# Lynx-MR/orbslam3lib

Measured on AMD Instinct MI355X. Metric: Mfeatures/s extract + Mmatches/s BFMatch, 640x480 stereo 8-level pyr, 1/2/4/8 GPU, higher is better.
Workload: dtype u8; 1 GPU; C2 640x480 stereo, 8 levels x1.2, 2000 feat/frame, FAST 20/7, + per-pair 2000x2000 Hamming kNN2 (left->right, all rows); parallelism=frames sharded across 1 GPU(s), replicas

## Files before the change

### orbslam3lib_amd/csrc/orb_kernels.hip

```cpp
#include <hip/hip_runtime.h>
#include <stdint.h>

#include <algorithm>
#include <atomic>

#include "orb_kernels.h"
#include "orb_math.h"
#include "orb_fast_cell.h"
#include "orb_octree.h"
#include "orb_pattern_data.h"
#include "orb_policy.h"

namespace orbgpu {

static_assert(sizeof(BatchArgs) <= 4096, "kernel argument block too large");

struct PatternTable {
    int8_t v[1024];
};
constexpr int hexval(char c) { return c <= '9' ? c - '0' : c - 'a' + 10; }
constexpr PatternTable make_pattern() {
    PatternTable t{};
    const char* h = ORBGPU_PATTERN_HEX;
    for (int i = 0; i < 1024; ++i) t.v[i] = (int8_t)(hexval(h[2 * i]) * 16 + hexval(h[2 * i + 1]));
// ... 923 lines not shown
        bool bad = false;
#pragma unroll
        for (int k = 0; k < kMaxLevels; ++k)
            if (k < a.nlevels) {
                if (k < l) out_row0 += a.lvlcnt[img * kMaxLevels + k];
                total += a.lvlcnt[img * kMaxLevels + k];
                bad |= a.status[img * kMaxLevels + k] != 0;
            }
        out_ok = !bad && total <= a.out_cap;
        if (bx == 0 && threadIdx.x == 0) {
            a.out_n[img] = bad ? -5 : total > a.out_cap ? -2 : total;
            a.out_mono[img] = out_ok ? total : 0;
        }
    }
    KP28* const out_kp = reinterpret_cast<KP28*>(a.out_kps) + (long long)img * a.out_cap + out_row0;
    uint8_t* const out_d = a.out_desc + ((long long)img * a.out_cap + out_row0) * 32;
    __shared__ __attribute__((aligned(16))) uint4 s_rng[17][17];
    __shared__ __attribute__((aligned(16))) uint4 s_pat[kOdPairs][kOdLanes];
    static_assert(kOdPairs * kOdLanes == 256 && 17 * 17 <= 2 * 256, "table copy: one / two entries per thread");
    const uint4* rng_src = reinterpret_cast<const uint4*>(c_od_tab.rng);
    const uint4 rng0 = rng_src[threadIdx.x];
    const uint4 pat0 = reinterpret_cast<const uint4*>(c_od_tab.pat)[threadIdx.x];
    if (threadIdx.x < 17 * 17 - 256) (&s_rng[0][0])[threadIdx.x + 256] = rng_src[threadIdx.x + 256];
    (&s_rng[0][0])[threadIdx.x] = rng0;
    (&s_pat[0][0])[threadIdx.x] = pat0;
    __syncthreads();
    int mv[3], mlo[3], mhi[3], mofs[3], mp16[3];
#pragma unroll
    for (int it = 0; it < 3; ++it) {
        const int i = sub + 32 * it, r = i / 3, part = i - 3 * r;
        mv[it] = r - 15;
        const int d = r < 31 ? c_umax[mv[it] < 0 ? -mv[it] : mv[it]] : -1;
        mlo[it] = 15 - d - 16 * part;
        mhi[it] = 16 + d - 16 * part;
        mofs[it] = (r < 31 ? mv[it] : 15) * G.pitch + 16 * part;
        mp16[it] = 16 * part;
    }
    const __amdgpu_buffer_rsrc_t lrs =
        __builtin_amdgcn_make_buffer_rsrc((void*)lvl, (short)0, (int)min((long long)G.pitch * G.h, 0x7fffffffLL), 0x00020000);
    uint8_t* pt = patch[grp];
    const int wave_first = (bx - G.od_first) * kOdKpBlock + (threadIdx.x >> 6) * 2;
    auto key_at = [&](int kb) {
        const int kp = kb + (grp & 1);
        return kp < count ? a.lvlkey[kbase + kp] : a.lvlkey[kbase + kb];
    };
    uint32_t key_next = wave_first < count ? key_at(wave_first) : 0u;
    for (int kb = wave_first; kb < count; kb += stride_k) {
        const int kp = kb + (grp & 1);
        const bool valid = kp < count;
        const uint32_t key = key_next;
        if (kb + stride_k < count) key_next = key_at(kb + stride_k);
        const int x = key_x(key) + kMinBorder, y = key_y(key) + kMinBorder;
        const int al = (x - 15) & 15;
        const int wofs = y * G.pitch + (x - 15 - al);
        uint4 mc[3];
#pragma unroll
        for (int it = 0; it < 3; ++it) {
            if (raw_dw) {
                const auto q = __builtin_amdgcn_raw_buffer_load_b128(lrs, wofs + mofs[it], 0, 0);
                mc[it] = make_uint4(q[0], q[1], q[2], q[3]);
            } else {
                const uint8_t* q = lvl + wofs + mofs[it];
                uint32_t d4[4];
#pragma unroll
                for (int k = 0; k < 4; ++k)
                    d4[k] = (uint32_t)q[4 * k] | ((uint32_t)q[4 * k + 1] << 8) | ((uint32_t)q[4 * k + 2] << 16) |
                            ((uint32_t)q[4 * k + 3] << 24);
                mc[it] = make_uint4(d4[0], d4[1], d4[2], d4[3]);
            }
        }
        const int xb = (x - kOdPatchR) & ~3;
        const int pofs = (y - kOdPatchR) * G.bpitch + xb;
        uint4 pv[kOdPatchIt];
#pragma unroll
        for (int it = 0; it < kOdPatchIt; ++it) {
            const int c = sub + it * kOdLanes;
            const int r = c / 3, part = c - 3 * r;
            if (c < kOdPatchChunks) {
                const auto q = __builtin_amdgcn_raw_buffer_load_b128(brs, pofs + r * G.bpitch + 16 * part, 0, 0);
                pv[it] = make_uint4(q[0], q[1], q[2], q[3]);
            }
        }
        int s_all = 0, c_all = 0, m01p = 0;
#pragma unroll
        for (int it = 0; it < 3; ++it) {
            const int m = min(max(mlo[it] + al, 0), 16), n = min(max(mhi[it] + al, 0), 16);
            const uint4 mk = s_rng[m][n];
            const uint32_t p0 = mc[it].x & mk.x, p1 = mc[it].y & mk.y, p2 = mc[it].z & mk.z, p3 = mc[it].w & mk.w;
            uint32_t sc = __builtin_amdgcn_udot4(p0, 0x01010101u, 0u, false);
            sc = __builtin_amdgcn_udot4(p1, 0x01010101u, sc, false);
            sc = __builtin_amdgcn_udot4(p2, 0x01010101u, sc, false);
            sc = __builtin_amdgcn_udot4(p3, 0x01010101u, sc, false);
            uint32_t cc = __builtin_amdgcn_udot4(p0, 0x03020100u, 0u, false);
            cc = __builtin_amdgcn_udot4(p1, 0x07060504u, cc, false);
            cc = __builtin_amdgcn_udot4(p2, 0x0B0A0908u, cc, false);
            cc = __builtin_amdgcn_udot4(p3, 0x0F0E0D0Cu, cc, false);
            s_all += (int)sc;
            c_all += (int)cc + mp16[it] * (int)sc;
            m01p += mv[it] * (int)sc;
        }
        const int m10 = od_sum(c_all - (15 + al) * s_all), m01 = od_sum(m01p);
        const float angle = fast_atan2_deg((float)m01, (float)m10);
        const float factorPI = (float)(3.14159265358979323846 / 180.0);
        float sn, ca;
        libm_sincosf(angle * factorPI, &sn, &ca);
#pragma unroll
        for (int it = 0; it < kOdPatchIt; ++it) {
            const int c = sub + it * kOdLanes;
            const int r = c / 3, part = c - 3 * r;
            if (c < kOdPatchChunks) *reinterpret_cast<uint4*>(pt + r * kOdPatchPitch + 16 * part) = pv[it];
        }
        __builtin_amdgcn_fence(__ATOMIC_RELEASE, "wavefront");
        __builtin_amdgcn_wave_barrier();
        __builtin_amdgcn_fence(__ATOMIC_ACQUIRE, "wavefront");
        const int pc = kOdPatchR * kOdPatchPitch + (x - xb);
        const float magic = 12582912.0f;
        const uint32_t kofs = (uint32_t)pc - 0x4B400000u - 0x400000u * (uint32_t)kOdPatchPitch;
        const f32x2 snv = {sn, sn}, cav = {ca, ca}, mg = {magic, magic};
        typedef const __attribute__((address_space(3))) uint8_t lds_u8;
        const uint32_t kpb = kofs + (uint32_t)(uintptr_t)(lds_u8*)pt;
        uint32_t bits = 0;
#pragma unroll
        for (int b = kOdPairs - 1; b >= 0; --b) {
            uint4 pw = s_pat[b][sub];
            asm volatile("" : "+v"(pw.x), "+v"(pw.y), "+v"(pw.z), "+v"(pw.w));
            const f32x2 X = {__uint_as_float(pw.x), __uint_as_float(pw.y)};
            const f32x2 Y = {__uint_as_float(pw.z), __uint_as_float(pw.w)};
            const f32x2 R = (X * snv + Y * cav) + mg;
            const f32x2 C = (X * cav - Y * snv) + mg;
            uint32_t m0 = __umul24(__float_as_uint(R.x), (uint32_t)kOdPatchPitch) + __float_as_uint(C.x);
            uint32_t m1 = __umul24(__float_as_uint(R.y), (uint32_t)kOdPatchPitch) + __float_as_uint(C.y);
            asm volatile("" : "+v"(m0), "+v"(m1));
            const uint32_t p0 = *(lds_u8*)(uintptr_t)(m0 + kpb), p1 = *(lds_u8*)(uintptr_t)(m1 + kpb);
            bits = __builtin_amdgcn_bitop3_b32(bits, (p0 - p1) >> (31 - b), 1u << b, 0xf8);
        }
        if (valid && !out_ok) {
            if (sub == 0) a.lvlangle[kbase + kp] = angle;
            a.lvldesc[(kbase + kp) * 32 + sub] = (uint8_t)bits;
        }
        if (valid) {
            if (out_ok) {
                out_d[kp * 32 + sub] = (uint8_t)bits;
                if (sub < 7) {
                    float px = (float)(x), py = (float)(y);
                    if (l != 0) {
                        px = px * G.scale;
                        py = py * G.scale;
                    }
                    const uint32_t w7[7] = {__float_as_uint(px), __float_as_uint(py), __float_as_uint((float)G.patch),
                                            __float_as_uint(angle), __float_as_uint((float)key_resp(key)),
                                            (uint32_t)l, 0xFFFFFFFFu};
                    uint32_t v = w7[0];
#pragma unroll
                    for (int k = 1; k < 7; ++k) v = sub == k ? w7[k] : v;
                    reinterpret_cast<uint32_t*>(out_kp + kp)[sub] = v;
                }
            }
        }
    }
}


constexpr int kFinU = 2;
#ifndef FIN_WIDE_MAX
#define FIN_WIDE_MAX 8
#endif
constexpr int kFinWideMaxImages = FIN_WIDE_MAX;

template <int kFinThreads>
__global__ __launch_bounds__(kFinThreads) void k_finalize(BatchArgs a) {
    __shared__ int4 s_lv[kMaxLevels];
    __shared__ int s_wave[2][kFinThreads / 64];
    const int img = a.img0 + blockIdx.x;
    const int tid = threadIdx.x, lane = tid & 63, w = tid >> 6;
    const int L = a.nlevels;
    int off[kMaxLevels];
    int total = 0;
    bool bad = false;
#pragma unroll
    for (int l = 0; l < kMaxLevels; ++l) {
        off[l] = total;
        if (l < L) {
            total += a.lvlcnt[img * kMaxLevels + l];
            bad |= a.status[img * kMaxLevels + l] != 0;
        }
    }
    if (bad || total > a.out_cap) {
        if (tid == 0) {
            a.out_n[img] = bad ? -5 : -2;
            a.out_mono[img] = 0;
        }
        return;
    }
    if (tid == 0) {
#pragma unroll
        for (int l = 0; l < kMaxLevels; ++l)
            if (l < L) s_lv[l] = make_int4(a.lv[l].kp_off, off[l], __float_as_int(l == 0 ? 1.f : a.lv[l].scale), a.lv[l].patch);
    }
    __syncthreads();
    const float lap0 = (float)a.laps[2 * img], lap1 = (float)a.laps[2 * img + 1];
    KP28* out = reinterpret_cast<KP28*>(a.out_kps) + (long long)img * a.out_cap;
    uint8_t* od = a.out_desc + (long long)img * a.out_cap * 32;
    const long long ibase = (long long)img * a.lvlkp_img_stride;
    const uint64_t lt = (1ull << lane) - 1ull;
    int mono = 0, stereo = 0, chunk_no = 0;
    for (int base = 0; base < total; base += kFinThreads * kFinU) {
        uint32_t key[kFinU];
        float ang[kFinU];
        uint4 d0[kFinU], d1[kFinU];
        int lev[kFinU];
#pragma unroll
        for (int u = 0; u < kFinU; ++u) {
            const int i = base + u * kFinThreads + tid;
            int l = 0;
#pragma unroll
            for (int k = 1; k < kMaxLevels; ++k) l += (k < L && i >= off[k]) ? 1 : 0;
            lev[u] = l;
            if (i < total) {
                const int4 info = s_lv[l];
                const long long kb = ibase + info.x + (i - info.y);
                key[u] = a.lvlkey[kb];
                ang[u] = a.lvlangle[kb];
                const uint4* s4 = reinterpret_cast<const uint4*>(a.lvldesc + kb * 32);
                d0[u] = s4[0];
                d1[u] = s4[1];
            }
        }
#pragma unroll
        for (int u = 0; u < kFinU; ++u) {
            const int cb = base + u * kFinThreads;
            if (cb >= total) continue;
            const int i = cb + tid;
            const bool valid = i < total;
            KP28 k;
            bool st = false;
            if (valid) {
                const int l = lev[u];
                const int4 info = s_lv[l];
                k.x = (float)(key_x(key[u]) + kMinBorder);
                k.y = (float)(key_y(key[u]) + kMinBorder);
                if (l != 0) {
                    k.x = k.x * __int_as_float(info.z);
                    k.y = k.y * __int_as_float(info.z);
                }
                k.size = (float)info.w;
                k.angle = ang[u];
                k.response = (float)key_resp(key[u]);
                k.octave = l;
                k.class_id = -1;
                st = (k.x >= lap0 && k.x <= lap1);
            }
            const uint64_t bal = __ballot(st);
            const int buf = chunk_no & 1;
            if (lane == 0) s_wave[buf][w] = __popcll(bal);
            __syncthreads();
            int before = 0, tst = 0;
#pragma unroll
            for (int v = 0; v < kFinThreads / 64; ++v) {
                const int c = s_wave[buf][v];
                tst += c;
                before += v < w ? c : 0;
            }
            const int exs = before + __popcll(bal & lt);
            const int exm = tid - exs;
            if (valid) {
                const int dst = st ? (total - 1 - (stereo + exs)) : (mono + exm);
                out[dst] = k;
                uint4* d4 = reinterpret_cast<uint4*>(od + (long long)dst * 32);
                d4[0] = d0[u];
                d4[1] = d1[u];
            }
            const int chunk = min(kFinThreads, total - cb);
            stereo += tst;
            mono += chunk - tst;
            ++chunk_no;
        }
    }
    if (threadIdx.x == 0) {
        a.out_n[img] = total;
        a.out_mono[img] = mono;
    }
}

__device__ inline uint32_t med3_u32(uint32_t a, uint32_t b, uint32_t c) {
    return max(min(a, b), min(max(a, b), c));
}

__device__ inline void knn2_store(uint32_t k1, uint32_t k2, int qi, int32_t* i1, int32_t* d1,
                                  int32_t* i2, int32_t* d2) {
    i1[qi] = k1 == 0xFFFFFFFFu ? -1 : (int32_t)(k1 & 0xFFFF);
    d1[qi] = k1 == 0xFFFFFFFFu ? 0x7fffffff : (int32_t)(k1 >> 16);
    i2[qi] = k2 == 0xFFFFFFFFu ? -1 : (int32_t)(k2 & 0xFFFF);
    d2[qi] = k2 == 0xFFFFFFFFu ? 0x7fffffff : (int32_t)(k2 >> 16);
}

typedef int knn_v8i __attribute__((ext_vector_type(8)));
typedef float knn_v16f __attribute__((ext_vector_type(16)));
constexpr int kKnnWaves = 8;
constexpr int kKnnThreads = 64 * kKnnWaves;
constexpr int kKnnQ = 32 * kKnnWaves;
static_assert(kKnnQ == kKnnQueries, "orb_kernels.h kKnnQueries (grid and arrival counters)");
constexpr int kKnnSeg = 4096;
constexpr int kKnnPitch4 = 144;
__device__ inline uint32_t knn_nib_of(uint32_t ws) {
    uint32_t r;
    asm("v_and_or_b32 %0, %1, %2, %3" : "=v"(r) : "v"(ws), "v"(0x88888888u), "v"(0x22222222u));
    return r;
}
__device__ inline knn_v8i knn4_expand(uint32_t w) {
    knn_v8i v;
    v[0] = (int)knn_nib_of(w << 3);
    v[1] = (int)knn_nib_of(w << 2);
    v[2] = (int)knn_nib_of(w << 1);
    v[3] = (int)knn_nib_of(w);
    v[4] = v[5] = v[6] = v[7] = 0;
    return v;
}
__device__ inline float knn_med3_f32(float a, float b, float c) {
    float r;
    asm("v_med3_f32 %0, %1, %2, %3" : "=v"(r) : "v"(a), "v"(b), "v"(c));
    return r;
}
__device__ inline float knn_max3_f32(float a, float b, float c) {
    float r;
    asm("v_max3_f32 %0, %1, %2, %3" : "=v"(r) : "v"(a), "v"(b), "v"(c));
    return r;
}
__device__ __attribute__((always_inline)) inline void knn2_fp4_block(
    const uint8_t* q, int nq, const uint8_t* t, int nt, int qb, int ts, int te, int32_t* i1, int32_t* d1,
    int32_t* i2, int32_t* d2, uint2* part, uint8_t* lds) {
    const int tid = threadIdx.x, lane = tid & 63, wave = tid >> 6;
    const int r = lane & 31, h = lane >> 5;
    const int qi = qb * kKnnQ + wave * 32 + r;
    knn_v8i qf[4];
    {
        const uint4* qp = reinterpret_cast<const uint4*>(q + (long long)min(qi, max(nq - 1, 0)) * 32);
        const uint4 qa = qp[0], qc = qp[1];
        qf[0] = knn4_expand(h ? qa.y : qa.x);
        qf[1] = knn4_expand(h ? qa.w : qa.z);
        qf[2] = knn4_expand(h ? qc.y : qc.x);
        qf[3] = knn4_expand(h ? qc.w : qc.z);
    }
    uint32_t g1 = 0xFFFFFFFFu, g2 = 0xFFFFFFFFu;
    const int er = tid >> 3, ed = tid & 7;
    const bool expander = tid < 256;
    auto load_packed = [&](int tile) __attribute__((always_inline)) {
        const int row = min(tile * 32 + er, nt - 1);
        return expander ? *reinterpret_cast<const uint32_t*>(t + (long long)row * 32 + 4 * ed) : 0u;
    };
    auto tile_lds = [&](int u) __attribute__((always_inline)) { return lds + ((u - ts) & 1) * (32 * kKnnPitch4); };
    auto store_expanded = [&](int u, uint32_t w) __attribute__((always_inline)) {
        if (expander) {
            const knn_v8i v = knn4_expand(w);
            *reinterpret_cast<uint4*>(tile_lds(u) + er * kKnnPitch4 + 16 * ed) = make_uint4(v[0], v[1], v[2], v[3]);
        }
    };
    uint32_t pk0 = 0, pk1 = 0;
    if (te > ts) {
        store_expanded(ts, load_packed(ts));
        pk1 = load_packed(ts + 1);
    }
    auto rowc = [](int g) { return (g & 3) + 8 * (g >> 2); };
    knn_v16f C0;
#pragma unroll
    for (int g = 0; g < 16; ++g) C0[g] = (float)(4095 - 4 * h - rowc(g));
    const float kNone = -1073741824.0f;
    for (int seg0 = (ts * 32 / kKnnSeg) * kKnnSeg; seg0 < te * 32; seg0 += kKnnSeg) {
        const int tile0 = max(seg0 >> 5, ts), tile1 = min(te, (seg0 + kKnnSeg) >> 5);
        float ka1 = kNone, ka2 = kNone, kb1 = kNone, kb2 = kNone;
        auto select = [&](const knn_v16f& v, bool shift) __attribute__((always_inline)) {
            if (shift) {
                ka1 += 32.f;
                ka2 += 32.f;
                kb1 += 32.f;
                kb2 += 32.f;
            }
#pragma unroll
            for (int g = 0; g < 16; g += 4) {
                const float x0 = v[g], y0 = v[g + 1], x1 = v[g + 2], y1 = v[g + 3];
                ka2 = fmaxf(ka2, knn_med3_f32(ka1, x0, y0));
                ka1 = knn_max3_f32(ka1, x0, y0);
                kb2 = fmaxf(kb2, knn_med3_f32(kb1, x1, y1));
                kb1 = knn_max3_f32(kb1, x1, y1);
            }
        };
        auto body = [&](int ti, auto par, knn_v16f& acc, const knn_v16f& prev) __attribute__((always_inline)) {
            constexpr int PAR = decltype(par)::value;
            uint32_t& pk_use = PAR ? pk0 : pk1;
            uint32_t& pk_load = PAR ? pk1 : pk0;
            __syncthreads();
            pk_load = load_packed(ti + 2);
            const uint8_t* ab = tile_lds(ti) + r * kKnnPitch4 + 16 * h;
#pragma unroll
            for (int s = 0; s < 4; ++s) {
                const uint4 a4 = *reinterpret_cast<const uint4*>(ab + 32 * s);
                const knn_v8i a = {(int)a4.x, (int)a4.y, (int)a4.z, (int)a4.w, 0, 0, 0, 0};
                acc = __builtin_amdgcn_mfma_scale_f32_32x32x64_f8f6f4(a, qf[s], s ? acc : C0, 4, 4, 0, 133, 0, 133);
            }
            if (ti > tile0) select(prev, ti - 1 > tile0);
            if (ti + 1 < te) store_expanded(ti + 1, pk_use);
            if (ti * 32 + 32 > nt) {
#pragma unroll
                for (int g = 0; g < 16; ++g)
                    if (ti * 32 + rowc(g) + 4 * h >= nt) acc[g] = kNone;
            }
        };
        using P0 = std::integral_constant<int, 0>;
        using P1 = std::integral_constant<int, 1>;
        knn_v16f acc0, acc1;
        int ti = tile0;
        for (; ti + 1 < tile1; ti += 2) {
            body(ti, P0{}, acc0, acc1);
            body(ti + 1, P1{}, acc1, acc0);
        }
        if (ti < tile1) {
            body(ti, P0{}, acc0, acc1);
            select(acc0, ti > tile0);
        } else if (tile1 > tile0) {
            select(acc1, tile1 - 1 > tile0);
        }
        const int unbias = 32 * (tile1 - 1 - tile0);
        const int k1 = (int)fmaxf(ka1, kb1) - unbias;
        const int k2 = (int)fmaxf(fminf(ka1, kb1), fmaxf(ka2, kb2)) - unbias;
        auto fold = [&](int k) __attribute__((always_inline)) {
            if (k < -(1 << 24)) return;
            const int tl = 4095 - (k & 4095), dotp = k >> 12;
            const uint32_t key = ((uint32_t)((256 - dotp) >> 1) << 16) | (uint32_t)(32 * tile0 + tl);
            g2 = med3_u32(g1, g2, key);
            g1 = min(g1, key);
        };
        fold(k1);
        fold(k2);
    }
    const uint32_t o1 = __shfl_xor(g1, 32), o2 = __shfl_xor(g2, 32);
    g2 = med3_u32(g1, g2, o1);
    g1 = min(g1, o1);
    g2 = med3_u32(g1, g2, o2);
    g1 = min(g1, o2);
    if (h == 0 && qi < nq) {
        if (part) part[qi] = make_uint2(g1, g2);
        else knn2_store(g1, g2, qi, i1, d1, i2, d2);
    }
}
constexpr int kKnnLdsBytes = 2 * 32 * kKnnPitch4;

__global__ __launch_bounds__(kKnnThreads) void k_knn2_mfma_pairs(MatchArgs m) {
    __shared__ __attribute__((aligned(16))) uint8_t lds[kKnnLdsBytes];
    const int pair = m.pair0 + blockIdx.y;
    const int qimg = 2 * pair, timg = 2 * pair + 1;
    const int qn = m.out_n[qimg], tn = m.out_n[timg];
    const int q0 = m.stereo_only ? m.out_mono[qimg] : 0;
    const int tq0 = m.stereo_only ? m.out_mono[timg] : 0;
    const int nq = qn > q0 ? qn - q0 : 0, nt = tn > tq0 ? tn - tq0 : 0;
    if (blockIdx.x == 0 && threadIdx.x == 0) m.nq[pair] = nq;
    if ((int)blockIdx.x * kKnnQ >= nq) return;
    const uint8_t* q = m.desc + ((long long)qimg * m.out_cap + q0) * 32;
    const uint8_t* t = m.desc + ((long long)timg * m.out_cap + tq0) * 32;
    const long long o = (long long)pair * m.out_cap;
    const int npt = (((nt + 31) >> 5) + 1) >> 1, S = gridDim.z, sp = blockIdx.z;
    const int ts = 2 * (npt * sp / S), te = min((nt + 31) >> 5, 2 * (npt * (sp + 1) / S));
    uint2* part = m.part ? m.part + ((long long)(blockIdx.y * S + sp)) * m.out_cap : nullptr;
    knn2_fp4_block(q, nq, t, nt, blockIdx.x, ts, te, m.idx1 + o, m.dist1 + o, m.idx2 + o, m.dist2 + o, part, lds);
    if (!part || !m.cnt || S == 1) return;
    asm volatile("s_waitcnt vmcnt(0)" ::: "memory");
    __syncthreads();
    int* s_last = reinterpret_cast<int*>(lds);
    if (threadIdx.x == 0) {
        uint32_t* c = m.cnt + blockIdx.y * gridDim.x + blockIdx.x;
        __builtin_amdgcn_fence(__ATOMIC_RELEASE, "agent");
        asm volatile("s_waitcnt vmcnt(0)" ::: "memory");
        const bool last = __hip_atomic_fetch_add(c, 1u, __ATOMIC_RELAXED, __HIP_MEMORY_SCOPE_AGENT) == (uint32_t)(S - 1);
        if (last) {
            __hip_atomic_store(c, 0u, __ATOMIC_RELAXED, __HIP_MEMORY_SCOPE_AGENT);
            __builtin_amdgcn_fence(__ATOMIC_ACQUIRE, "agent");
            asm volatile("s_waitcnt vmcnt(0)" ::: "memory");
        }
        *s_last = last ? 1 : 0;
    }
    __syncthreads();
    if (!*s_last) return;
    const long long pb = (long long)blockIdx.y * S * m.out_cap;
    for (int i = threadIdx.x; i < kKnnQ; i += kKnnThreads) {
        const int qi = blockIdx.x * kKnnQ + i;
        if (qi >= nq) break;
        uint32_t g1 = 0xFFFFFFFFu, g2 = 0xFFFFFFFFu;
        for (int k = 0; k < S; ++k) {
            const uint2 kk = m.part[pb + (long long)k * m.out_cap + qi];
            g2 = med3_u32(g1, g2, kk.x);
            g1 = min(g1, kk.x);
            g2 = med3_u32(g1, g2, kk.y);
            g1 = min(g1, kk.y);
        }
        knn2_store(g1, g2, qi, m.idx1 + o, m.dist1 + o, m.idx2 + o, m.dist2 + o);
    }
}

__global__ __launch_bounds__(256) void k_knn2_merge(MatchArgs m, int nsplit) {
    const int pair = m.pair0 + blockIdx.y;
    const int qimg = 2 * pair, timg = 2 * pair + 1;
    const int qn = m.out_n[qimg], tn = m.out_n[timg];
    const int q0 = m.stereo_only ? m.out_mono[qimg] : 0;
    const int nq = qn > q0 ? qn - q0 : 0;
    (void)tn;
    const int qi = blockIdx.x * 256 + threadIdx.x;
    if (qi >= nq) return;
    uint32_t g1 = 0xFFFFFFFFu, g2 = 0xFFFFFFFFu;
    for (int sp = 0; sp < nsplit; ++sp) {
        const uint2 k = m.part[((long long)(blockIdx.y * nsplit + sp)) * m.out_cap + qi];
        g2 = med3_u32(g1, g2, k.x);
        g1 = min(g1, k.x);
        g2 = med3_u32(g1, g2, k.y);
        g1 = min(g1, k.y);
    }
    const long long o = (long long)pair * m.out_cap;
    knn2_store(g1, g2, qi, m.idx1 + o, m.dist1 + o, m.idx2 + o, m.dist2 + o);
}

__global__ __launch_bounds__(kKnnThreads) void k_knn2_mfma_plain(const uint8_t* q, int nq, const uint8_t* t, int nt,
                                                         int32_t* i1, int32_t* d1, int32_t* i2, int32_t* d2) {
    __shared__ __attribute__((aligned(16))) uint8_t lds[kKnnLdsBytes];
    knn2_fp4_block(q, nq, t, nt, blockIdx.x, 0, (nt + 31) >> 5, i1, d1, i2, d2, nullptr, lds);
}

hipError_t launch_blur_level(const BatchArgs& a, int l, hipStream_t s) {
    const LevelGeom G = a.lv[l];
    const int n = G.tiles_x * G.tiles_y;
    hipLaunchKernelGGL(k_blur, dim3(std::min(n * a.nimages, 8192)), dim3(256), 0, s, a, G.tile_first, n);
    return hipGetLastError();
}
void fast_cell_range(const BatchArgs& a, int tile, int* c0, int* c1) {
    const int s48 = a.fast_n48, s64 = a.fast_n64;
    *c0 = tile == kCellPitchTiny ? 0 : tile == kCellPitchSmall ? s48 : s64;
    *c1 = tile == kCellPitchTiny ? s48 : tile == kCellPitchSmall ? s64 : a.total_cells;
}
hipError_t launch_fast_cells(const BatchArgs& a, int tile, hipStream_t s) {
    int c0, c1;
    fast_cell_range(a, tile, &c0, &c1);
    const bool merge = a.nimages <= kFastMergeMaxImages && a.fast_small <= 0 && a.fast_n48 > 0 && a.fast_n64 > a.fast_n48;
    if (merge && tile == kCellPitchSmall) return hipSuccess;
    if (merge && tile == kCellPitchTiny) {
        tile = kCellPitchSmall;
        c1 = a.fast_n64;
    }
    if (c1 <= c0) return hipSuccess;
    const dim3 grid(c1 - c0, a.nimages);
    const dim3 block(tile == kCellPitchTiny ? fast_threads<kCellPitchTiny>() : tile == kCellPitchSmall ? fast_threads<kCellPitchSmall>()
                                                                                                      : fast_threads<kCellMax>());
    const uint32_t d = (uint32_t)(c1 - c0);
    const uint32_t magic = d > 1 ? 0xFFFFFFFFu / d + 1u : 0u;
    const bool small = (tile == kCellPitchTiny || tile == kCellPitchSmall) && a.fast_ovf &&
                       (a.fast_small > 0 || (a.fast_small < 0 && a.nimages > kFastMergeMaxImages));
    const dim3 oblock(fast_threads<kCellPitchSmall>());
    if (small && tile == kCellPitchTiny) {
        hipLaunchKernelGGL((k_fast_cells<kCellPitchTiny, true>), grid, block, 0, s, a, c0, magic);
        int d0, d1;
        fast_cell_range(a, kCellPitchSmall, &d0, &d1);
        if (d1 <= d0) hipLaunchKernelGGL(k_fast_cells_ovf<kCellPitchSmall>, dim3(kFastOvfBlocks), oblock, 0, s, a);
    } else if (small) {
        hipLaunchKernelGGL((k_fast_cells<kCellPitchSmall, true>), grid, block, 0, s, a, c0, magic);
        hipLaunchKernelGGL(k_fast_cells_ovf<kCellPitchSmall>, dim3(kFastOvfBlocks), oblock, 0, s, a);
    } else if (tile == kCellPitchTiny) hipLaunchKernelGGL((k_fast_cells<kCellPitchTiny, false>), grid, block, 0, s, a, c0, magic);
    else if (tile == kCellPitchSmall) hipLaunchKernelGGL((k_fast_cells<kCellPitchSmall, false>), grid, block, 0, s, a, c0, magic);
    else hipLaunchKernelGGL((k_fast_cells<kCellMax, false>), grid, block, 0, s, a, c0, magic);
    return hipGetLastError();
}
hipError_t launch_octree(const BatchArgs& a, hipStream_t s) {
    constexpr int kMaxDevices = 64;
    static std::atomic<int> lds_set[kMaxDevices];
    int dev = 0;
    if (hipGetDevice(&dev) != hipSuccess || dev < 0 || dev >= kMaxDevices) dev = kMaxDevices - 1;
    std::atomic<int>& set = lds_set[dev];
    if (a.oct_lds_bytes > 65536 && a.oct_lds_bytes > set.load()) {
        for (const void* f : {reinterpret_cast<const void*>(k_octree<512>),
                              reinterpret_cast<const void*>(k_octree_retry)}) {
            hipError_t e = hipFuncSetAttribute(f, hipFuncAttributeMaxDynamicSharedMemorySize, a.oct_lds_bytes);
            if (e != hipSuccess) return e;
        }
        int cur = set.load();
        while (a.oct_lds_bytes > cur && !set.compare_exchange_weak(cur, a.oct_lds_bytes)) {}
    }
    const int split = a.nimages < a.oct_split_min_images ? a.nlevels : std::min(a.oct_split, a.nlevels);
    if (split > 0)
        hipLaunchKernelGGL(k_octree<512>, dim3(a.nimages, split), dim3(512), a.oct_lds_bytes, s, a, 0,
                           OctCfg{a.oct_nq_off, a.oct_lds_nodes, kOctLdsKeys, a.oct_lds_bytes});
    if (split < a.nlevels) {
        const OctCfg q{a.oct2_nq_off, a.oct2_lds_nodes, a.oct2_lds_keys, a.oct2_lds_bytes};
        if (a.oct2_threads == 128)
            hipLaunchKernelGGL(k_octree<128>, dim3(a.nimages, a.nlevels - split), dim3(128), a.oct2_lds_bytes, s, a,
                               split, q);
        else
            hipLaunchKernelGGL(k_octree<256>, dim3(a.nimages, a.nlevels - split), dim3(256), a.oct2_lds_bytes, s, a,
                               split, q);
    }
    if (a.oct_may_retry)
        hipLaunchKernelGGL(k_octree_retry, dim3(std::min(a.nimages * a.nlevels, 64)), dim3(512),
                           a.oct_lds_bytes, s, a);
    return hipGetLastError();
}
hipError_t launch_orient_desc(const BatchArgs& a, hipStream_t s) {
    const uint32_t d = (uint32_t)a.total_od_blocks;
    const uint32_t magic = d > 1 ? 0xFFFFFFFFu / d + 1u : 0u;
    hipLaunchKernelGGL(k_orient_desc, dim3(a.total_od_blocks, a.nimages), dim3(256), 0, s, a, magic);
    return hipGetLastError();
}
hipError_t launch_finalize(const BatchArgs& a, hipStream_t s) {
    if (a.nimages <= 2) hipLaunchKernelGGL(k_finalize<1024>, dim3(a.nimages), dim3(1024), 0, s, a);
    else if (a.nimages <= kFinWideMaxImages) hipLaunchKernelGGL(k_finalize<512>, dim3(a.nimages), dim3(512), 0, s, a);
    else hipLaunchKernelGGL(k_finalize<256>, dim3(a.nimages), dim3(256), 0, s, a);
    return hipGetLastError();
}
hipError_t launch_knn2_pairs(const MatchArgs& m, int npairs, hipStream_t s) {
    const int S = m.part ? std::max(1, std::min(kKnnMaxSplit, kKnnSplitSlots / std::max(npairs, 1))) : 1;
    const int qblocks = (m.out_cap + kKnnQ - 1) / kKnnQ;
    if (S > 1) {
        if (npairs * S > kKnnSplitSlots || (m.cnt && (long long)npairs * qblocks > m.cnt_slots))
            return hipErrorInvalidValue;
        hipLaunchKernelGGL(k_knn2_mfma_pairs, dim3(qblocks, npairs, S), dim3(kKnnThreads), 0, s, m);
        if (!m.cnt) hipLaunchKernelGGL(k_knn2_merge, dim3((m.out_cap + 255) / 256, npairs), dim3(256), 0, s, m, S);
        return hipGetLastError();
    }
    MatchArgs m1 = m;
    m1.part = nullptr;
    hipLaunchKernelGGL(k_knn2_mfma_pairs, dim3(qblocks, npairs), dim3(kKnnThreads), 0, s, m1);
    return hipGetLastError();
}
hipError_t launch_knn2_plain(const uint8_t* q, int nq, const uint8_t* t, int nt, int32_t* i1,
                             int32_t* d1, int32_t* i2, int32_t* d2, hipStream_t s) {
    if (nq == 0) return hipSuccess;
    hipLaunchKernelGGL(k_knn2_mfma_plain, dim3((nq + kKnnQ - 1) / kKnnQ), dim3(kKnnThreads), 0, s, q, nq, t, nt, i1,
                       d1, i2, d2);
    return hipGetLastError();
}

}
```

Baseline: 576.7 Mfeatures/s.

## Stage four key tiles per LDS buffer and software-pipeline kNN fragment reads

The FP4 MFMA Hamming kNN kernel now expands 128 train rows (four 32-row tiles) per barrier instead of one tile. All 512 threads take part in expansion instead of 256, and LDS fragments for the next tile are read ahead while the current MFMAs run. The split across partitions is aligned to stages, the ragged-tail masking is reworked, and waves_per_eu(4) is added to steer register allocation. The aim is fewer __syncthreads and better overlap of LDS and global loads with MFMA work, at the cost of more LDS, more registers and masked work in padded tail tiles.

```diff
diff --git a/orbslam3lib_amd/csrc/orb_kernels.hip b/orbslam3lib_amd/csrc/orb_kernels.hip
--- a/orbslam3lib_amd/csrc/orb_kernels.hip
+++ b/orbslam3lib_amd/csrc/orb_kernels.hip
@@ -1249,6 +1249,11 @@
 static_assert(kKnnQ == kKnnQueries, "orb_kernels.h kKnnQueries (grid and arrival counters)");
 constexpr int kKnnSeg = 4096;
 constexpr int kKnnPitch4 = 144;
+constexpr int kKnnStageTiles = 4;
+constexpr int kKnnStageRows = 32 * kKnnStageTiles;
+constexpr int kKnnStageBytes = kKnnStageRows * kKnnPitch4;
+constexpr int kKnnLdsBytes = 2 * kKnnStageBytes;
+static_assert(kKnnSeg % kKnnStageRows == 0, "a key segment is whole stages");
 __device__ inline uint32_t knn_nib_of(uint32_t ws) {
     uint32_t r;
     asm("v_and_or_b32 %0, %1, %2, %3" : "=v"(r) : "v"(ws), "v"(0x88888888u), "v"(0x22222222u));
@@ -1290,38 +1295,38 @@
     }
     uint32_t g1 = 0xFFFFFFFFu, g2 = 0xFFFFFFFFu;
     const int er = tid >> 3, ed = tid & 7;
-    const bool expander = tid < 256;
-    auto load_packed = [&](int tile) __attribute__((always_inline)) {
-        const int row = min(tile * 32 + er, nt - 1);
-        return expander ? *reinterpret_cast<const uint32_t*>(t + (long long)row * 32 + 4 * ed) : 0u;
+    auto load_packed = [&](int stage, int half) __attribute__((always_inline)) {
+        const int row = min(stage * kKnnStageRows + 64 * half + er, nt - 1);
+        return stage * kKnnStageTiles < te ? *reinterpret_cast<const uint32_t*>(t + (uint32_t)(row * 32 + 4 * ed)) : 0u;
     };
-    auto tile_lds = [&](int u) __attribute__((always_inline)) { return lds + ((u - ts) & 1) * (32 * kKnnPitch4); };
-    auto store_expanded = [&](int u, uint32_t w) __attribute__((always_inline)) {
-        if (expander) {
-            const knn_v8i v = knn4_expand(w);
-            *reinterpret_cast<uint4*>(tile_lds(u) + er * kKnnPitch4 + 16 * ed) = make_uint4(v[0], v[1], v[2], v[3]);
-        }
+    auto store_expanded = [&](int stage, uint32_t w0, uint32_t w1) __attribute__((always_inline)) {
+        uint8_t* d = lds + (stage & 1) * kKnnStageBytes + er * kKnnPitch4 + 16 * ed;
+        const knn_v8i v = knn4_expand(w0), w = knn4_expand(w1);
+        *reinterpret_cast<uint4*>(d) = make_uint4(v[0], v[1], v[2], v[3]);
+        *reinterpret_cast<uint4*>(d + 64 * kKnnPitch4) = make_uint4(w[0], w[1], w[2], w[3]);
     };
     uint32_t pk0 = 0, pk1 = 0;
     if (te > ts) {
-        store_expanded(ts, load_packed(ts));
-        pk1 = load_packed(ts + 1);
+        const int j0 = ts / kKnnStageTiles;
+        store_expanded(j0, load_packed(j0, 0), load_packed(j0, 1));
+        pk0 = load_packed(j0 + 1, 0);
+        pk1 = load_packed(j0 + 1, 1);
     }
     auto rowc = [](int g) { return (g & 3) + 8 * (g >> 2); };
     knn_v16f C0;
 #pragma unroll
     for (int g = 0; g < 16; ++g) C0[g] = (float)(4095 - 4 * h - rowc(g));
     const float kNone = -1073741824.0f;
+    const int row_end = min(te * 32, nt);
     for (int seg0 = (ts * 32 / kKnnSeg) * kKnnSeg; seg0 < te * 32; seg0 += kKnnSeg) {
         const int tile0 = max(seg0 >> 5, ts), tile1 = min(te, (seg0 + kKnnSeg) >> 5);
+        const int tile_end = (tile1 + kKnnStageTiles - 1) / kKnnStageTiles * kKnnStageTiles;
         float ka1 = kNone, ka2 = kNone, kb1 = kNone, kb2 = kNone;
-        auto select = [&](const knn_v16f& v, bool shift) __attribute__((always_inline)) {
-            if (shift) {
-                ka1 += 32.f;
-                ka2 += 32.f;
-                kb1 += 32.f;
-                kb2 += 32.f;
-            }
+        auto select = [&](const knn_v16f& v) __attribute__((always_inline)) {
+            ka1 += 32.f;
+            ka2 += 32.f;
+            kb1 += 32.f;
+            kb2 += 32.f;
 #pragma unroll
             for (int g = 0; g < 16; g += 4) {
                 const float x0 = v[g], y0 = v[g + 1], x1 = v[g + 2], y1 = v[g + 3];
@@ -1331,42 +1336,47 @@
                 kb1 = knn_max3_f32(kb1, x1, y1);
             }
         };
-        auto body = [&](int ti, auto par, knn_v16f& acc, const knn_v16f& prev) __attribute__((always_inline)) {
-            constexpr int PAR = decltype(par)::value;
-            uint32_t& pk_use = PAR ? pk0 : pk1;
-            uint32_t& pk_load = PAR ? pk1 : pk0;
+        knn_v16f acc0, acc1;
+#pragma unroll
+        for (int g = 0; g < 16; ++g) acc1[g] = kNone;
+        for (int j = tile0 / kKnnStageTiles; j * kKnnStageTiles < tile_end; ++j) {
             __syncthreads();
-            pk_load = load_packed(ti + 2);
-            const uint8_t* ab = tile_lds(ti) + r * kKnnPitch4 + 16 * h;
-#pragma unroll
-            for (int s = 0; s < 4; ++s) {
-                const uint4 a4 = *reinterpret_cast<const uint4*>(ab + 32 * s);
-                const knn_v8i a = {(int)a4.x, (int)a4.y, (int)a4.z, (int)a4.w, 0, 0, 0, 0};
-                acc = __builtin_amdgcn_mfma_scale_f32_32x32x64_f8f6f4(a, qf[s], s ? acc : C0, 4, 4, 0, 133, 0, 133);
-            }
-            if (ti > tile0) select(prev, ti - 1 > tile0);
-            if (ti + 1 < te) store_expanded(ti + 1, pk_use);
-            if (ti * 32 + 32 > nt) {
-#pragma unroll
-                for (int g = 0; g < 16; ++g)
-                    if (ti * 32 + rowc(g) + 4 * h >= nt) acc[g] = kNone;
-            }
-        };
-        using P0 = std::integral_constant<int, 0>;
-        using P1 = std::integral_constant<int, 1>;
-        knn_v16f acc0, acc1;
-        int ti = tile0;
-        for (; ti + 1 < tile1; ti += 2) {
-            body(ti, P0{}, acc0, acc1);
-            body(ti + 1, P1{}, acc1, acc0);
-        }
-        if (ti < tile1) {
-            body(ti, P0{}, acc0, acc1);
-            select(acc0, ti > tile0);
-        } else if (tile1 > tile0) {
-            select(acc1, tile1 - 1 > tile0);
-        }
-        const int unbias = 32 * (tile1 - 1 - tile0);
+            if ((j + 1) * kKnnStageTiles < te) store_expanded(j + 1, pk0, pk1);
+            pk0 = load_packed(j + 2, 0);
+            pk1 = load_packed(j + 2, 1);
+            __builtin_amdgcn_sched_barrier(0);
+            const uint8_t* ab = lds + (j & 1) * kKnnStageBytes + r * kKnnPitch4 + 16 * h;
+            const bool ragged = (j + 1) * kKnnStageRows > row_end;
+            uint4 fr[2][4];
+            auto read_frags = [&](int k) __attribute__((always_inline)) {
+#pragma unroll
+                for (int s = 0; s < 4; ++s)
+                    fr[k & 1][s] = *reinterpret_cast<const uint4*>(ab + k * (32 * kKnnPitch4) + 32 * s);
+            };
+            read_frags(0);
+#pragma unroll
+            for (int k = 0; k < kKnnStageTiles; ++k) {
+                knn_v16f& acc = (k & 1) ? acc1 : acc0;
+                const knn_v16f& prev = (k & 1) ? acc0 : acc1;
+                const uint4* f = fr[k & 1];
+                if (k + 1 < kKnnStageTiles) read_frags(k + 1);
+#pragma unroll
+                for (int s = 0; s < 4; ++s) {
+                    const knn_v8i a = {(int)f[s].x, (int)f[s].y, (int)f[s].z, (int)f[s].w, 0, 0, 0, 0};
+                    acc = __builtin_amdgcn_mfma_scale_f32_32x32x64_f8f6f4(a, qf[s], s ? acc : C0, 4, 4, 0, 133, 0, 133);
+                }
+                select(prev);
+                if (ragged) {
+                    const float lim = (float)(4095 - (row_end - (j * kKnnStageTiles + k) * 32));
+#pragma unroll
+                    for (int g = 0; g < 16; ++g)
+                        if (C0[g] <= lim) acc[g] = kNone;
+                }
+                __builtin_amdgcn_sched_barrier(0);
+            }
+        }
+        if (tile_end > tile0) select(acc1);
+        const int unbias = 32 * (tile_end - 1 - tile0);
         const int k1 = (int)fmaxf(ka1, kb1) - unbias;
         const int k2 = (int)fmaxf(fminf(ka1, kb1), fmaxf(ka2, kb2)) - unbias;
         auto fold = [&](int k) __attribute__((always_inline)) {
@@ -1389,9 +1399,9 @@
         else knn2_store(g1, g2, qi, i1, d1, i2, d2);
     }
 }
-constexpr int kKnnLdsBytes = 2 * 32 * kKnnPitch4;
-
-__global__ __launch_bounds__(kKnnThreads) void k_knn2_mfma_pairs(MatchArgs m) {
+static_assert(kKnnThreads * 2 * 4 == kKnnStageRows * 32, "two packed dwords per thread and stage");
+
+__global__ __launch_bounds__(kKnnThreads) __attribute__((amdgpu_waves_per_eu(4))) void k_knn2_mfma_pairs(MatchArgs m) {
     __shared__ __attribute__((aligned(16))) uint8_t lds[kKnnLdsBytes];
     const int pair = m.pair0 + blockIdx.y;
     const int qimg = 2 * pair, timg = 2 * pair + 1;
@@ -1404,8 +1414,8 @@
     const uint8_t* q = m.desc + ((long long)qimg * m.out_cap + q0) * 32;
     const uint8_t* t = m.desc + ((long long)timg * m.out_cap + tq0) * 32;
     const long long o = (long long)pair * m.out_cap;
-    const int npt = (((nt + 31) >> 5) + 1) >> 1, S = gridDim.z, sp = blockIdx.z;
-    const int ts = 2 * (npt * sp / S), te = min((nt + 31) >> 5, 2 * (npt * (sp + 1) / S));
+    const int nst = (nt + kKnnStageRows - 1) / kKnnStageRows, S = gridDim.z, sp = blockIdx.z;
+    const int ts = kKnnStageTiles * (nst * sp / S), te = min((nt + 31) >> 5, kKnnStageTiles * (nst * (sp + 1) / S));
     uint2* part = m.part ? m.part + ((long long)(blockIdx.y * S + sp)) * m.out_cap : nullptr;
     knn2_fp4_block(q, nq, t, nt, blockIdx.x, ts, te, m.idx1 + o, m.dist1 + o, m.idx2 + o, m.dist2 + o, part, lds);
     if (!part || !m.cnt || S == 1) return;
@@ -1463,7 +1473,7 @@
     knn2_store(g1, g2, qi, m.idx1 + o, m.dist1 + o, m.idx2 + o, m.dist2 + o);
 }
 
-__global__ __launch_bounds__(kKnnThreads) void k_knn2_mfma_plain(const uint8_t* q, int nq, const uint8_t* t, int nt,
+__global__ __launch_bounds__(kKnnThreads) __attribute__((amdgpu_waves_per_eu(4))) void k_knn2_mfma_plain(const uint8_t* q, int nq, const uint8_t* t, int nt,
                                                          int32_t* i1, int32_t* d1, int32_t* i2, int32_t* d2) {
     __shared__ __attribute__((aligned(16))) uint8_t lds[kKnnLdsBytes];
     knn2_fp4_block(q, nq, t, nt, blockIdx.x, 0, (nt + 31) >> 5, i1, d1, i2, d2, nullptr, lds);
```

Result: no change. 574.3 Mfeatures/s (-0.4%).
